# fabsig/GPBoost

Measured on AMD Instinct MI355X. Metric: neg-log-lik evals/sec, n=1000000 Vecchia(m=30) fp64, higher is better.
Workload: dtype f64

## Files before the change

### gpboost_amd/csrc/dev_common.h

```cpp
#pragma once
#include <hip/hip_runtime.h>
#include <stdint.h>
#include <type_traits>
#include <utility>

namespace gpb {

template <int B, int E, class F>
__device__ __forceinline__ void static_for(F&& f) {
  if constexpr (B < E) {
    f(std::integral_constant<int, B>{});
    static_for<B + 1, E>(f);
  }
}
template <int B, int E, class F>
__device__ __forceinline__ void static_for_down(F&& f) {
  if constexpr (B < E) {
    f(std::integral_constant<int, E - 1>{});
    static_for_down<B, E - 1>(f);
  }
}

template <int LANE>
__device__ __forceinline__ double row_bcast(double x) {
  static_assert(LANE >= 0 && LANE < 16, "row_newbcast lane");
  double r;
  asm volatile("s_nop 1\n\tv_mov_b64_dpp %0, %1 row_newbcast:%2 row_mask:0xf bank_mask:0xf"
               : "=v"(r)
               : "v"(x), "n"(LANE));
  return r;
}
template <int LANE>
__device__ __forceinline__ void row_fnma(double& acc, double b, double own) {
  static_assert(LANE >= 0 && LANE < 16, "row_newbcast lane");
#ifdef GPB_DPP_PAD_EVERY_FMAC
  asm volatile("s_nop 1\n\tv_fmac_f64_dpp %0, -%1, %2 row_newbcast:%3 row_mask:0xf bank_mask:0xf"
               : "+v"(acc)
               : "v"(b), "v"(own), "n"(LANE));
#else
  asm volatile("v_fmac_f64_dpp %0, -%1, %2 row_newbcast:%3 row_mask:0xf bank_mask:0xf"
               : "+v"(acc)
               : "v"(b), "v"(own), "n"(LANE));
#endif
}
__device__ __forceinline__ void dpp_fence(double& a) { asm volatile("s_nop 1" : "+v"(a)); }
__device__ __forceinline__ void dpp_fence(double& a, double& b) { asm volatile("s_nop 1" : "+v"(a), "+v"(b)); }
__device__ __forceinline__ void dpp_fence(double& a, double& b, double& c) { asm volatile("s_nop 1" : "+v"(a), "+v"(b), "+v"(c)); }
__device__ __forceinline__ void dpp_fence(double& a, double& b, double& c, double& d) { asm volatile("s_nop 1" : "+v"(a), "+v"(b), "+v"(c), "+v"(d)); }
template <int CTRL>
__device__ __forceinline__ double dpp_move_f64(double v) {
  const long long b = __builtin_bit_cast(long long, v);
  int lo = (int)(b & 0xffffffffll), hi = (int)(b >> 32);
  lo = __builtin_amdgcn_update_dpp(0, lo, CTRL, 0xF, 0xF, true);
  hi = __builtin_amdgcn_update_dpp(0, hi, CTRL, 0xF, 0xF, true);
  return __builtin_bit_cast(double, ((long long)hi << 32) | (long long)(unsigned int)lo);
}
__device__ __forceinline__ double row_sum16(double v) {
  v += dpp_move_f64<0xB1>(v);
  v += dpp_move_f64<0x4E>(v);
  v += dpp_move_f64<0x141>(v);
  v += dpp_move_f64<0x140>(v);
  return v;
}
__host__ __device__ constexpr unsigned long long row_lanes_le(int j) {
  return j < 0 ? 0ull : (j >= 15 ? ~0ull : ((1ull << (j + 1)) - 1ull) * 0x0001000100010001ull);
}
__host__ __device__ constexpr unsigned long long row_lane_eq(int j) { return (1ull << j) * 0x0001000100010001ull; }
template <unsigned long long MASK>
__device__ __forceinline__ int sel_lanes(int a, int b, int tok) {
  int r;
  asm("s_mov_b32 vcc_lo, %3\n\ts_mov_b32 vcc_hi, %4\n\tv_cndmask_b32_e32 %0, %1, %2, vcc ; %5"
      : "=v"(r) : "v"(b), "v"(a), "n"((int)(unsigned)(MASK & 0xffffffffull)), "n"((int)(unsigned)(MASK >> 32)), "s"(tok) : "vcc");
  return r;
}
template <unsigned long long MASK, int A, int B>
__device__ __forceinline__ int sel_lanes_const(int tok) {
  static_assert(A >= 0 && A <= 64 && B >= 0 && B <= 64, "inline constants only");
  int r;
  asm("s_mov_b32 vcc_lo, %3\n\ts_mov_b32 vcc_hi, %4\n\tv_cndmask_b32_e64 %0, %1, %2, vcc ; %5"
      : "=v"(r) : "n"(B), "n"(A), "n"((int)(unsigned)(MASK & 0xffffffffull)), "n"((int)(unsigned)(MASK >> 32)), "s"(tok) : "vcc");
  return r;
}
template <unsigned long long MASK>
__device__ __forceinline__ void set_lanes(double& dst, double v) {
  asm volatile("s_mov_b32 exec_lo, %2\n\ts_mov_b32 exec_hi, %3\n\tv_mov_b64 %0, %1\n\ts_mov_b64 exec, -1"
               : "+v"(dst) : "v"(v), "n"((int)(unsigned)(MASK & 0xffffffffull)), "n"((int)(unsigned)(MASK >> 32)));
}
template <int LANE>
__device__ __forceinline__ double row_bcast_builtin(double x) {
  const long long v = __builtin_bit_cast(long long, x);
  int lo = (int)(v & 0xffffffffll), hi = (int)(v >> 32);
  lo = __builtin_amdgcn_update_dpp(0, lo, 0x150 + LANE, 0xf, 0xf, false);
  hi = __builtin_amdgcn_update_dpp(0, hi, 0x150 + LANE, 0xf, 0xf, false);
  const long long r = ((long long)hi << 32) | (unsigned long long)(unsigned int)lo;
  return __builtin_bit_cast(double, r);
}
#ifdef GPB_DPP_VIA_BUILTIN
#define GPB_ROW_BCAST(L, x) ::gpb::row_bcast_builtin<L>(x)
#define GPB_ROW_FNMA(L, acc, b, own) (acc) = __builtin_fma(-::gpb::row_bcast_builtin<L>(b), (own), (acc))
#else
#define GPB_ROW_BCAST(L, x) ::gpb::row_bcast<L>(x)
#define GPB_ROW_FNMA(L, acc, b, own) ::gpb::row_fnma<L>((acc), (b), (own))
#endif


__device__ __forceinline__ double fast_rcp(double x) {
  const double y0 = __builtin_amdgcn_rcp(x);
  const double e = __builtin_fma(-x, y0, 1.0);
  return __builtin_fma(y0, e, y0);
}

#ifndef GPB_EXP_TAB_SIZE
#define GPB_EXP_TAB_SIZE 256
#endif
static_assert(GPB_EXP_TAB_SIZE == 256, "exp_of_scaled is written for a 256-entry table");

enum CovType : int { kMatern05 = 0, kMatern15 = 1, kMatern25 = 2 };

constexpr double kLn2OverT = 0.0027076061740622863;
constexpr double kCoordScale = 184.6649652337873;

struct KernEval { double ev, rp; };
__device__ __forceinline__ KernEval exp_of_scaled(double d2q, const double* __restrict__ tabv) {
  const double h = __builtin_amdgcn_rsq(d2q);
  const double g = d2q * h;
  const double e = __builtin_fma(-h, g, 3.0);
  const double rp = g * e;
  const double kf = __builtin_rint(-rp);
  const double rr = -rp - kf;
  const int k = (int)kf;
  double p = __builtin_fma(rr, 2.239395190875157e-12, 3.3083026805413713e-09);
  p = __builtin_fma(p, rr, 3.6655655969101062e-06);
  p = __builtin_fma(p, rr, kLn2OverT);
  p = __builtin_fma(p, rr, 1.0);
  KernEval o;
  o.ev = __builtin_ldexp(tabv[k & (GPB_EXP_TAB_SIZE - 1)] * p, k >> 8);
  o.rp = rp;
  return o;
}
template <int COV>
__device__ __forceinline__ double matern_cov_s(double d2s, const double* __restrict__ tabv) {
  const KernEval k = exp_of_scaled(d2s, tabv);
  if constexpr (COV == kMatern05) return k.ev;
  else if constexpr (COV == kMatern15) return k.ev * __builtin_fma(k.rp, kLn2OverT, 1.0);
  else { const double r = k.rp * kLn2OverT; return k.ev * __builtin_fma(r, __builtin_fma(r, 1.0 / 3.0, 1.0), 1.0); }
}
template <int COV>
__device__ __forceinline__ double matern_cov_dlog_s(double d2s, const double* __restrict__ tabv, double& dk) {
  const KernEval k = exp_of_scaled(d2s, tabv);
  const double r = k.rp * kLn2OverT;
  if constexpr (COV == kMatern05) { dk = -r * k.ev; return k.ev; }
  else if constexpr (COV == kMatern15) { dk = -(r * r) * k.ev; return k.ev * (1.0 + r); }
  else { dk = -(1.0 / 3.0) * (r * r) * (1.0 + r) * k.ev; return k.ev * __builtin_fma(r, __builtin_fma(r, 1.0 / 3.0, 1.0), 1.0); }
}
template <int COV>
__device__ __forceinline__ double matern_dlog_range_s(double d2s, const double* __restrict__ tabv) {
  const KernEval k = exp_of_scaled(d2s, tabv);
  const double r = k.rp * kLn2OverT;
  if constexpr (COV == kMatern05) return -r * k.ev;
  else if constexpr (COV == kMatern15) return -(r * r) * k.ev;
  else return -(1.0 / 3.0) * (r * r) * __builtin_fma(1.0, r, 1.0) * k.ev;
}

}
```

### gpboost_amd/csrc/vecchia_kernels.hip

```cpp
#include <algorithm>
#include "dev_common.h"
#include "vecchia_kernels.h"

namespace gpb {

namespace {

constexpr double kDummyCoord = 1e30;

__host__ __device__ constexpr int lane_of_row(int r) { return ((r / 16) & 1) ? 15 - (r % 16) : (r % 16); }

template <int MT>
struct Layout {
  static_assert(MT >= 1 && MT <= 62, "1 <= MT <= 62");
  static_assert(MT % 16 != 15, "row MT and row MT+1 must share a register slot");
  static constexpr int R = MT + 2;
  static constexpr int NS = (R + 15) / 16;
  static constexpr int PS = MT / 16, PL = lane_of_row(MT);
  static constexpr int YS = (MT + 1) / 16, YL = lane_of_row(MT + 1);
  static constexpr int NCOL = MT + 1;
  static constexpr int PTS_BYTES32 = (NS * 16) * 32 + 16;
  static constexpr int PTS_STRIDE24 = NS * 16 + 2;
  __host__ __device__ static constexpr int cmax(int s) { return (16 * s + 15 < MT) ? 16 * s + 15 : MT; }
};

template <bool D3> struct RecT;
template <> struct RecT<true> { double x, y, z, w; __device__ __forceinline__ double zz() const { return z; } };
template <> struct RecT<false> { double x, y, w; __device__ __forceinline__ double zz() const { return 0.0; } };

template <bool D3>
__device__ __forceinline__ double sq_dist_s(double px, double py, double pz, double qx, double qy, double qz) {
  const double dx = px - qx, dy = py - qy;
  double d2 = __builtin_fma(dx, dx, 1e-300);
  d2 = __builtin_fma(dy, dy, d2);
  if constexpr (D3) {
    const double dz = pz - qz;
    d2 = __builtin_fma(dz, dz, d2);
  }
  return d2;
}

template <int MT>
__host__ __device__ constexpr int num_lower_steps() {
  using L = Layout<MT>;
  int n = 8 * L::NS * (L::NS - 1) + 15 * (L::NS / 2);
  if (L::NS & 1) { const int s = L::NS - 1; const int chi = (16 * s + 14 < MT - 1) ? 16 * s + 14 : MT - 1; n += chi - 16 * s + 1; }
  return n;
}
template <int MT, class FR, class FP, class FS>
__device__ __forceinline__ void for_each_lower_step(FR&& rect, FP&& pair, FS&& solo) {
  using L = Layout<MT>;
  constexpr int RECT_TOTAL = 8 * L::NS * (L::NS - 1);
  static_for<1, L::NS>([&](auto s_) {
    constexpr int s = decltype(s_)::value;
    static_for<0, 16 * s>([&](auto c_) { rect(s_, c_, std::integral_constant<int, 8 * s * (s - 1) + decltype(c_)::value>{}); });
  });
  static_for<0, L::NS>([&](auto s_) {
    constexpr int s = decltype(s_)::value;
    if constexpr ((s & 1) == 1) {
      static_for<0, 15>([&](auto j_) {
        constexpr int j = decltype(j_)::value;
        constexpr int cA = 16 * s + j, cB = 16 * (s - 1) + 14 - j;
        using E = std::integral_constant<int, RECT_TOTAL + 15 * (s / 2) + j>;
        if constexpr (cA <= MT - 1) pair(s_, std::integral_constant<int, cA>{}, std::integral_constant<int, s - 1>{},
                                         std::integral_constant<int, cB>{}, std::integral_constant<int, 14 - j>{}, E{});
        else solo(std::integral_constant<int, s - 1>{}, std::integral_constant<int, cB>{}, E{});
      });
    } else if constexpr (s == L::NS - 1) {
      constexpr int chi = (16 * s + 14 < MT - 1) ? 16 * s + 14 : MT - 1;
      static_for<16 * s, chi + 1>([&](auto c_) { solo(s_, c_, std::integral_constant<int, RECT_TOTAL + 15 * (L::NS / 2) + decltype(c_)::value - 16 * s>{}); });
    }
  });
}

}

constexpr unsigned long long kGranuleEmpty = ~0ull;
template <int NP>
__device__ __forceinline__ void vecchia_finish(const VecchiaKernelArgs& args, int G, double (*s_fin)[4]);

template <int MT, int MODE>
constexpr bool kRuntimeWeightedInstance() { return MODE == MODE_GRAD && MT > 30 && MT <= 40; }

template <int MT, int COV, bool D3, int MODE, bool WT>
__global__ __launch_bounds__(256, (MT > 30 && MT <= 40 && MODE != MODE_NLL) ? 2 : 1) void vecchia_point_kernel(VecchiaKernelArgs args) {
  using L = Layout<MT>;
  constexpr int NS = L::NS;
  constexpr bool kNeedSolve = (MODE != MODE_NLL);
#ifdef GPB_NLL_RIGHT_LOOKING
  constexpr bool kLeftLooking = false;
#else
  constexpr bool kLeftLooking = MT > 30 && (!kNeedSolve || NS == 3);
#endif
  constexpr bool kLeftSolve = kLeftLooking && kNeedSolve;
  constexpr int NP = (MODE == MODE_GRAD) ? GPB_NUM_PARTIALS : 3;

  using Rec = RecT<D3>;
  constexpr bool kStoreDK = (MODE == MODE_GRAD) && (MT <= 30);
  constexpr int NSTEP = num_lower_steps<MT>();
  constexpr bool kLastDkInReg = kStoreDK && D3;
  constexpr int NSTORE = kStoreDK ? (kLastDkInReg ? NSTEP - 1 : NSTEP) : 1;
  constexpr int PBYTES = D3 ? L::PTS_BYTES32 : L::PTS_STRIDE24 * (int)sizeof(Rec);
  __shared__ double s_tab[GPB_EXP_TAB_SIZE];
  __shared__ __attribute__((aligned(16))) char s_pts_raw[16 * PBYTES];
  __shared__ double s_red[GPB_NUM_PARTIALS][16];
  __shared__ double s_f0[kLeftSolve ? 16 : 1][kLeftSolve ? 256 : 1];
  constexpr bool kDgInLds = WT && (MODE == MODE_NLL) && kLeftLooking;
  __shared__ double s_dg[kDgInLds ? 16 : 1][kDgInLds ? NS * 16 : 1];
  __shared__ double s_dk[NSTORE][kStoreDK ? 256 : 1];
  static_assert(PBYTES % 16 == 0 && PBYTES >= 16 * (NS * 16), "record block: 16-byte aligned, room for the (A, b) pairs");
  __shared__ double2 s_ab[(MODE == MODE_GRAD && !kStoreDK) ? 16 : 1][(MODE == MODE_GRAD && !kStoreDK) ? NS * 16 : 1];
  double dk_last = 0.0;

  __shared__ double s_tot[GPB_NUM_PARTIALS];
  __shared__ double s_fin[GPB_NUM_PARTIALS][4];

  const int G = (int)gridDim.x - 1;
  if ((int)blockIdx.x == G) { vecchia_finish<NP>(args, G, s_fin); return; }
  const int tid0 = threadIdx.x;
  static_assert(GPB_EXP_TAB_SIZE == 256, "one table entry per thread");
  s_tab[tid0] = args.exp_tab[tid0] * args.var;
  if (tid0 < NP) s_tot[tid0] = 0.0;
  __shared__ double s_pm[16];
  __shared__ int s_pe[16];
  if (tid0 < 16) { s_pm[tid0] = 0.5; s_pe[tid0] = 1; }

  const int m = args.m;
  auto fetch_idx = [&](int grp_, int tid_, int (&out)[NS]) {
    const int g_ = tid_ >> 4, l_ = tid_ & 15;
    const long long ir = (long long)args.i_begin + (long long)grp_ * 16 + g_;
    const int ii = ir < (long long)args.i_end ? (int)ir : args.i_end - 1;
#pragma unroll
    for (int s = 0; s < NS; ++s) {
      const int r = 16 * s + ((s & 1) ? 15 - l_ : l_);
      int idx = -1;
      if (r < m) idx = args.nn[(size_t)ii * m + r];
      else if (r == MT) idx = ii;
      out[s] = idx;
    }
  };
  int nidx[NS];
  fetch_idx(blockIdx.x, tid0, nidx);
  for (int grp = blockIdx.x; grp < args.ngroups; grp += G) {
  int tid = tid0;
  asm volatile("; per-trip thread index" : "+v"(tid));
  const int g = tid >> 4;
  const int l = tid & 15;
  const long long i_raw = (long long)args.i_begin + (long long)grp * 16 + g;
  const bool active = i_raw < (long long)args.i_end;
  const int i = active ? (int)i_raw : args.i_end - 1;
  int cidx[NS];
#pragma unroll
  for (int s = 0; s < NS; ++s) cidx[s] = nidx[s];
  if (grp + G < args.ngroups) fetch_idx(grp + G, tid, nidx);
  const double sc = args.a * kCoordScale;

  const double4 ctr = args.pts[i];
  Rec own[NS];
  constexpr bool kRuntimeW = WT && kRuntimeWeightedInstance<MT, MODE>();
  const bool weighted = kRuntimeW ? (args.nug != nullptr) : WT;
  constexpr int kOwnDg = (kDgInLds || !WT) ? 1 : NS;
  double own_dg[kOwnDg];
#pragma unroll
  for (int s = 0; s < kOwnDg; ++s) own_dg[s] = 0.0;
  auto own_dg_of = [&](int s) -> double { if constexpr (kOwnDg == NS) return own_dg[s]; else { (void)s; return own_dg[0]; } };
#pragma unroll
  for (int s = 0; s < NS; ++s) {
    const int r = 16 * s + ((s & 1) ? 15 - l : l);
    const int idx = cidx[s];
    if (WT && weighted) {
      const double dgv = args.var + (idx >= 0 ? args.nug[idx] : 1.0);
      if constexpr (kDgInLds) s_dg[g][r] = dgv; else own_dg[s] = dgv;
    }
    Rec p;
    if (idx >= 0) {
      const double4 q = args.pts[idx];
      p.x = (q.x - ctr.x) * sc; p.y = (q.y - ctr.y) * sc; p.w = q.w;
      if constexpr (D3) p.z = (q.z - ctr.z) * sc;
    } else {
      p.x = kDummyCoord * (double)(r + 1); p.y = 0.0; p.w = 0.0;
      if constexpr (D3) p.z = 0.0;
    }
    own[s] = p;
    reinterpret_cast<Rec*>(s_pts_raw + g * PBYTES)[r] = p;
  }
  __syncthreads();
  const double* tabv = s_tab;
  const Rec* gp = reinterpret_cast<const Rec*>(s_pts_raw + g * PBYTES);
  int row_off[NS];
#pragma unroll
  for (int s = 0; s < NS; ++s) row_off[s] = (16 * s + ((s & 1) ? 15 - l : l)) * (int)sizeof(Rec);

  double M[NS][L::NCOL];
  auto eval_entry = [&](const Rec& o, const Rec& q, auto e_) -> double {
    const double d2 = sq_dist_s<D3>(o.x, o.y, o.zz(), q.x, q.y, q.zz());
    if constexpr (kStoreDK) {
      double dk;
      const double v = matern_cov_dlog_s<COV>(d2, tabv, dk);
      if constexpr (kLastDkInReg && decltype(e_)::value == NSTEP - 1) dk_last = dk;
      else s_dk[decltype(e_)::value][tid] = dk;
      return v;
    } else {
      return matern_cov_s<COV>(d2, tabv);
    }
  };
  if constexpr (kLeftLooking) {
    auto eval_plain = [&](const Rec& o, const Rec& q) -> double {
      return matern_cov_s<COV>(sq_dist_s<D3>(o.x, o.y, o.zz(), q.x, q.y, q.zz()), tabv);
    };
    static_for<0, MT + 1>([&](auto c_) {
      constexpr int c = decltype(c_)::value;
      constexpr int sc_ = c / 16, lc = lane_of_row(c);
      if constexpr (c < MT) {
        static_for<sc_ + 1, NS>([&](auto s_) { constexpr int s = decltype(s_)::value; M[s][c] = eval_plain(own[s], gp[c]); });
        if constexpr ((c % 16) != 15 && (sc_ & 1) == 0) {
          constexpr int j = 14 - (c - 16 * sc_);
          constexpr int sA = sc_ + 1, cA = 16 * sA + j;
          if constexpr (sA < NS && cA <= MT - 1) {
            constexpr unsigned long long MA = row_lanes_le(14 - j);
            const int ro = sel_lanes<MA>(row_off[sA], row_off[sc_], grp);
            const int co = sel_lanes_const<MA, cA, c>(grp) * (int)sizeof(Rec);
            const double v = eval_plain(*reinterpret_cast<const Rec*>(reinterpret_cast<const char*>(gp) + ro),
                                        *reinterpret_cast<const Rec*>(reinterpret_cast<const char*>(gp) + co));
            M[sA][cA] = v;
            M[sc_][c] = v;
          } else {
            M[sc_][c] = eval_plain(own[sc_], gp[c]);
          }
        }
      }
      {
        double dg;
        if constexpr (kDgInLds) dg = weighted ? s_dg[g][c] : ((c == MT) ? args.diag_i : args.diag_nn);
        else dg = weighted ? own_dg_of(sc_) : ((c == MT) ? args.diag_i : args.diag_nn);
        if constexpr (c == 16 * sc_ + 15 || c == MT) M[sc_][c] = dg;
        else set_lanes<row_lane_eq(lc)>(M[sc_][c], dg);
        set_lanes<row_lane_eq(L::YL)>(M[L::YS][c], gp[c].w);
      }
      static_for<0, c>([&](auto k_) {
        constexpr int k = decltype(k_)::value;
        static_for<sc_, NS>([&](auto s_) {
          constexpr int s = decltype(s_)::value;
          GPB_ROW_FNMA(lc, M[s][c], M[sc_][k], M[s][k]);
        });
      });
      if constexpr (c < MT) {
        const double piv = GPB_ROW_BCAST(lc, M[sc_][c]);
        const double y0 = __builtin_amdgcn_rsq(piv);
        const double e = __builtin_fma(-0.5 * piv * y0, y0, 0.5);
        const double rs = __builtin_fma(y0, e, y0);
        static_for<sc_, NS>([&](auto s_) { constexpr int s = decltype(s_)::value; M[s][c] *= rs; });
        if constexpr (kLeftSolve) set_lanes<row_lane_eq(lc)>(M[sc_][c], rs);
        static_assert(NS <= 4, "dpp_fence overloads cover four slots");
        if constexpr (NS - sc_ == 1) dpp_fence(M[sc_][c]);
        else if constexpr (NS - sc_ == 2) dpp_fence(M[sc_][c], M[sc_ + 1][c]);
        else if constexpr (NS - sc_ == 3) dpp_fence(M[sc_][c], M[sc_ + 1][c], M[sc_ + 2][c]);
        else dpp_fence(M[sc_][c], M[sc_ + 1][c], M[sc_ + 2][c], M[sc_ + 3][c]);
        if constexpr (kLeftSolve && c == 15) static_for<0, 16>([&](auto q_) { s_f0[decltype(q_)::value][tid] = M[0][decltype(q_)::value]; });
      }
    });
  } else {
  for_each_lower_step<MT>(
      [&](auto s_, auto c_, auto e_) {
        constexpr int s = decltype(s_)::value, c = decltype(c_)::value;
        M[s][c] = eval_entry(own[s], gp[c], e_);
      },
      [&](auto sA_, auto cA_, auto sB_, auto cB_, auto J_, auto e_) {
        constexpr int sA = decltype(sA_)::value, cA = decltype(cA_)::value, sB = decltype(sB_)::value,
                      cB = decltype(cB_)::value, J = decltype(J_)::value;
        constexpr unsigned long long MA = row_lanes_le(J);
        const int ro = sel_lanes<MA>(row_off[sA], row_off[sB], grp);
        const int co = sel_lanes_const<MA, cA, cB>(grp) * (int)sizeof(Rec);
        const Rec o = *reinterpret_cast<const Rec*>(reinterpret_cast<const char*>(gp) + ro);
        const Rec q = *reinterpret_cast<const Rec*>(reinterpret_cast<const char*>(gp) + co);
        const double v = eval_entry(o, q, e_);
        M[sA][cA] = v;
        M[sB][cB] = v;
      },
      [&](auto s_, auto c_, auto e_) {
        constexpr int s = decltype(s_)::value, c = decltype(c_)::value;
        M[s][c] = eval_entry(own[s], gp[c], e_);
      });
  static_for<0, NS>([&](auto s_) {
    constexpr int s = decltype(s_)::value;
    static_for<16 * s, L::cmax(s) + 1>([&](auto c_) {
      constexpr int c = decltype(c_)::value;
      double dg;
      if constexpr (kDgInLds) dg = weighted ? s_dg[g][c] : ((c == MT) ? args.diag_i : args.diag_nn);
      else dg = weighted ? own_dg_of(s) : ((c == MT) ? args.diag_i : args.diag_nn);
      if constexpr (c == 16 * s + 15 || c == MT) M[s][c] = dg;
      else set_lanes<row_lane_eq(lane_of_row(c))>(M[s][c], dg);
    });
  });
  if (l == L::YL) {
    static_for<0, MT + 1>([&](auto c_) { M[L::YS][decltype(c_)::value] = gp[decltype(c_)::value].w; });
  }

  static_for<0, MT>([&](auto k_) {
    constexpr int k = decltype(k_)::value;
    constexpr int sk = k / 16, lk = lane_of_row(k);
    if constexpr (k == 0) static_for<0, NS>([&](auto s_) { dpp_fence(M[decltype(s_)::value][0]); });
    const double piv = GPB_ROW_BCAST(lk, M[sk][k]);
    const double inv = fast_rcp(piv);
    double T[NS];
    static_for<sk, NS>([&](auto s_) { T[decltype(s_)::value] = M[decltype(s_)::value][k] * inv; });
    static_for<k + 1, MT + 1>([&](auto c_) {
      constexpr int c = decltype(c_)::value;
      constexpr int sc_ = c / 16, lc = lane_of_row(c);
      static_for<sc_, NS>([&](auto s_) {
        constexpr int s = decltype(s_)::value;
        GPB_ROW_FNMA(lc, M[s][c], M[sc_][k], T[s]);
      });
    });
    if constexpr (kNeedSolve) static_for<sk, NS>([&](auto s_) { M[decltype(s_)::value][k] = T[decltype(s_)::value]; });
  });
  }

  const double Dv = GPB_ROW_BCAST(L::PL, M[L::PS][MT]);
  const double uv = GPB_ROW_BCAST(L::YL, M[L::YS][MT]);
  const double Dinv = 1.0 / Dv;

  double red[GPB_NUM_PARTIALS];
#pragma unroll
  for (int t = 0; t < GPB_NUM_PARTIALS; ++t) red[t] = 0.0;
  red[GPB_P_LOGDET] = Dv;
  red[GPB_P_QUAD] = uv * uv * Dinv;
  red[GPB_P_BAD] = (Dv > 0.0) ? 0.0 : 1.0;

  if constexpr (kNeedSolve) {
    constexpr bool kLaneX = MT > 30;
    double X[kLaneX ? 1 : MT];
    double xa[NS], xb[NS];
    if constexpr (kLeftSolve) {
      static_assert(NS == 3 && L::PS == 2 && L::YS == 2, "kLeftSolve: three slots, the point's and the response row in the last one");
#pragma unroll
      for (int s = 0; s < NS; ++s) { xa[s] = 0.0; xb[s] = 0.0; }
      static_for_down<0, MT>([&](auto k_) {
        constexpr int k = decltype(k_)::value;
        constexpr int sk = k / 16, lk = lane_of_row(k);
        constexpr unsigned long long kKeep = (sk & 1) ? row_lanes_le(14 - (k % 16)) : ~row_lanes_le(k % 16);
        double own_col;
        if constexpr (sk == 0) own_col = s_f0[k][tid]; else own_col = M[sk][k];
        double ta = own_col * xa[sk], tb = own_col * xb[sk];
        set_lanes<~kKeep>(ta, 0.0);
        set_lanes<~kKeep>(tb, 0.0);
        static_for<sk + 1, NS>([&](auto s_) {
          constexpr int s = decltype(s_)::value;
          ta = __builtin_fma(M[s][k], xa[s], ta);
          tb = __builtin_fma(M[s][k], xb[s], tb);
        });
        ta = row_sum16(ta); tb = row_sum16(tb);
        const double rk = GPB_ROW_BCAST(lk, own_col);
        const double la = GPB_ROW_BCAST(L::PL, M[L::PS][k]);
        const double lb = GPB_ROW_BCAST(L::YL, M[L::YS][k]);
        set_lanes<row_lane_eq(lk)>(xa[sk], (la - ta) * rk);
        set_lanes<row_lane_eq(lk)>(xb[sk], (lb - tb) * rk);
      });
    } else if constexpr (kLaneX) {
#pragma unroll
      for (int s = 0; s < NS; ++s) { xa[s] = 0.0; xb[s] = 0.0; }
      static_for_down<0, MT>([&](auto k_) {
        constexpr int k = decltype(k_)::value;
        constexpr int sk = k / 16, lk = lane_of_row(k);
        constexpr unsigned long long kKeep = (sk & 1) ? row_lanes_le(14 - (k % 16)) : ~row_lanes_le(k % 16);
        double ta = M[sk][k] * xa[sk], tb = M[sk][k] * xb[sk];
        set_lanes<~kKeep>(ta, 0.0);
        set_lanes<~kKeep>(tb, 0.0);
        static_for<sk + 1, NS>([&](auto s_) {
          constexpr int s = decltype(s_)::value;
          ta = __builtin_fma(M[s][k], xa[s], ta);
          tb = __builtin_fma(M[s][k], xb[s], tb);
        });
        ta = row_sum16(ta); tb = row_sum16(tb);
        const double la = GPB_ROW_BCAST(L::PL, M[L::PS][k]);
        const double lb = GPB_ROW_BCAST(L::YL, M[L::YS][k]);
        set_lanes<row_lane_eq(lk)>(xa[sk], la - ta);
        set_lanes<row_lane_eq(lk)>(xb[sk], lb - tb);
      });
    } else {
    static_for<0, MT>([&](auto k_) { X[decltype(k_)::value] = M[L::PS][decltype(k_)::value]; });
    static_for<0, MT>([&](auto k_) { static_for<0, NS>([&](auto s_) { if constexpr (decltype(k_)::value <= L::cmax(decltype(s_)::value)) dpp_fence(M[decltype(s_)::value][decltype(k_)::value]); }); });
    static_for_down<0, MT>([&](auto j_) {
      constexpr int j = decltype(j_)::value;
      constexpr int sj = j / 16, lj = lane_of_row(j);
      static_for_down<0, j>([&](auto k_) {
        constexpr int k = decltype(k_)::value;
        GPB_ROW_FNMA(lj, X[k], M[sj][k], X[j]);
      });
    });
    }
    if constexpr (MODE == MODE_FACTOR) {
      if constexpr (kLaneX) {
        if (active) {
          double* Arow = args.A + (size_t)i * m;
#pragma unroll
          for (int s = 0; s < NS; ++s) { const int r = 16 * s + ((s & 1) ? 15 - l : l); if (r < m) Arow[r] = xa[s]; }
        }
      } else {
      if (active && l == L::PL) {
        double* Arow = args.A + (size_t)i * m;
        static_for<0, MT>([&](auto k_) {
          constexpr int k = decltype(k_)::value;
          if (k < m) Arow[k] = X[k];
        });
      }
      }
      if (active && l == 0) { args.D[i] = Dv; args.u[i] = uv; }
    }
    if constexpr (MODE == MODE_GRAD) {
      asm volatile("" ::: "memory");
      double2* gab = kStoreDK ? reinterpret_cast<double2*>(s_pts_raw + g * PBYTES) : &s_ab[g][0];
      if constexpr (kLaneX) {
#pragma unroll
        for (int s = 0; s < NS; ++s) {
          const int r = 16 * s + ((s & 1) ? 15 - l : l);
          gab[r] = r < MT ? make_double2(xa[s], xb[s]) : (r == MT ? make_double2(-1.0, 0.0) : make_double2(0.0, 0.0));
        }
      } else {
      if (l == L::PL) { static_for<0, MT>([&](auto k_) { gab[decltype(k_)::value].x = X[decltype(k_)::value]; }); gab[MT].x = -1.0; gab[MT + 1].x = 0.0; }
      if (l == L::YL) { static_for<0, MT>([&](auto k_) { gab[decltype(k_)::value].y = X[decltype(k_)::value]; }); gab[MT].y = 0.0; gab[MT + 1].y = 0.0; }
      if (l == 0) { for (int r = MT + 2; r < NS * 16; ++r) gab[r] = make_double2(0.0, 0.0); }
      }
      __syncthreads();
      double2 abr[NS];
      int ab_off[NS];
      double sAA = 0.0, sbA = 0.0;
      static_for<0, NS>([&](auto s_) {
        constexpr int s = decltype(s_)::value;
        const int r = 16 * s + ((s & 1) ? 15 - l : l);
        abr[s] = gab[r]; ab_off[s] = r * (int)sizeof(double2);
        const double nr = weighted ? own_dg_of(s) - args.var : 1.0;
        if (r < MT) { sAA = __builtin_fma(nr * abr[s].x, abr[s].x, sAA); sbA = __builtin_fma(nr * abr[s].y, abr[s].x, sbA); }
      });
      double accD = 0.0, accU = 0.0;
      auto accumulate = [&](double dk, const double2& r_, const double2& c_) {
        accD = __builtin_fma(dk * r_.x, c_.x, accD);
        accU = __builtin_fma(dk, __builtin_fma(r_.y, c_.x, c_.y * r_.x), accU);
      };
      auto dk_of = [&](auto e_, const Rec& o, const Rec& q) -> double {
        if constexpr (kStoreDK) {
          if constexpr (kLastDkInReg && decltype(e_)::value == NSTEP - 1) return dk_last;
          else return s_dk[decltype(e_)::value][tid];
        } else {
          return matern_dlog_range_s<COV>(sq_dist_s<D3>(o.x, o.y, o.zz(), q.x, q.y, q.zz()), tabv);
        }
      };
      for_each_lower_step<MT>(
          [&](auto s_, auto c_, auto e_) {
            constexpr int s = decltype(s_)::value, c = decltype(c_)::value;
            if constexpr (kStoreDK) accumulate(dk_of(e_, own[s], gp[c]), abr[s], gab[c]);
            else accumulate(dk_of(e_, *reinterpret_cast<const Rec*>(reinterpret_cast<const char*>(gp) + row_off[s]), gp[c]), abr[s], gab[c]);
          },
          [&](auto sA_, auto cA_, auto sB_, auto cB_, auto J_, auto e_) {
            constexpr int sA = decltype(sA_)::value, cA = decltype(cA_)::value, sB = decltype(sB_)::value,
                          cB = decltype(cB_)::value, J = decltype(J_)::value;
            constexpr unsigned long long MA = row_lanes_le(J);
            const int ci = sel_lanes_const<MA, cA, cB>(grp);
            double dk;
            if constexpr (kStoreDK) dk = dk_of(e_, own[0], own[0]);
            else {
              const int ro = sel_lanes<MA>(row_off[sA], row_off[sB], grp);
              dk = dk_of(e_, *reinterpret_cast<const Rec*>(reinterpret_cast<const char*>(gp) + ro),
                         *reinterpret_cast<const Rec*>(reinterpret_cast<const char*>(gp) + ci * (int)sizeof(Rec)));
            }
            const int ao = sel_lanes<MA>(ab_off[sA], ab_off[sB], grp);
            accumulate(dk, *reinterpret_cast<const double2*>(reinterpret_cast<const char*>(gab) + ao), gab[ci]);
          },
          [&](auto s_, auto c_, auto e_) {
            constexpr int s = decltype(s_)::value, c = decltype(c_)::value;
            static_assert((s & 1) == 0, "solo steps only occur in even slots");
            double dk;
            if constexpr (kStoreDK) dk = dk_of(e_, own[s], gp[c]);
            else dk = dk_of(e_, *reinterpret_cast<const Rec*>(reinterpret_cast<const char*>(gp) + row_off[s]), gp[c]);
            set_lanes<row_lanes_le(c - 16 * s)>(dk, 0.0);
            accumulate(dk, abr[s], gab[c]);
          });
#pragma unroll
      for (int off = 8; off >= 1; off >>= 1) {
        accD += __shfl_xor(accD, off, 16);
        accU += __shfl_xor(accU, off, 16);
        sAA += __shfl_xor(sAA, off, 16);
        sbA += __shfl_xor(sbA, off, 16);
      }
      const double up = uv * Dinv;
      double nug_i = args.nugget;
      if (WT && weighted) nug_i = args.nug[i];
      const double dD_var = Dv - nug_i - sAA;
      const double uk_var = -sbA;
      const double dD_rng = 2.0 * accD;
      const double uk_rng = accU;
      red[GPB_P_G1_VAR] = uk_var * up - 0.5 * up * up * dD_var;
      red[GPB_P_G2_VAR] = 0.5 * Dinv * dD_var;
      red[GPB_P_G1_RNG] = uk_rng * up - 0.5 * up * up * dD_rng;
      red[GPB_P_G2_RNG] = 0.5 * Dinv * dD_rng;
    }
  }

  if (l == 0) {
#pragma unroll
    for (int t = 0; t < NP; ++t) s_red[t][g] = active ? red[t] : (t == GPB_P_LOGDET ? 1.0 : 0.0);
  }
  __syncthreads();
  if (tid < 16) {
    const double dv = s_red[GPB_P_LOGDET][tid];
    const double p = s_pm[tid] * __builtin_amdgcn_frexp_mant(dv);
    s_pm[tid] = (dv > 0.0) ? __builtin_amdgcn_frexp_mant(p) : __builtin_nan("");
    s_pe[tid] += __builtin_amdgcn_frexp_exp(dv) + __builtin_amdgcn_frexp_exp(p);
  } else if (tid >= 64 && tid < 64 + NP && tid - 64 != GPB_P_LOGDET) {
    const int t = tid - 64;
    double acc = 0.0;
#pragma unroll
    for (int q = 0; q < 16; ++q) acc += s_red[t][q];
    s_tot[t] += acc;
  }
  }
  const int tid = tid0;
  __syncthreads();
  if (tid < 16) s_red[GPB_P_LOGDET][tid] = log(s_pm[tid]) + (double)s_pe[tid] * 0.693147180559945309417232121458;
  __syncthreads();
  if (tid == 0) {
    double acc = 0.0;
#pragma unroll
    for (int q = 0; q < 16; ++q) acc += s_red[GPB_P_LOGDET][q];
    s_tot[GPB_P_LOGDET] = acc;
  }
  __syncthreads();

  if (tid < NP)
    __hip_atomic_store(reinterpret_cast<unsigned long long*>(args.partials + (size_t)tid * G + blockIdx.x),
                       (unsigned long long)__double_as_longlong(s_tot[tid]), __ATOMIC_RELAXED, __HIP_MEMORY_SCOPE_AGENT);
}

template <int NP>
__device__ __forceinline__ void vecchia_finish(const VecchiaKernelArgs& args, int G, double (*s_fin)[4]) {
  const int tid = threadIdx.x;
#pragma unroll
  for (int t = 0; t < NP; ++t) {
    double acc = 0.0, comp = 0.0;
    unsigned long long* base = reinterpret_cast<unsigned long long*>(args.partials + (size_t)t * G);
    constexpr int kBatch = 8;
    for (int b0 = tid; b0 < G; b0 += 256 * kBatch) {
      unsigned long long raw[kBatch];
#pragma unroll
      for (int q = 0; q < kBatch; ++q) {
        const int b = b0 + 256 * q;
        raw[q] = b < G ? __hip_atomic_load(base + b, __ATOMIC_RELAXED, __HIP_MEMORY_SCOPE_AGENT) : 0ull;
      }
#pragma unroll
      for (int q = 0; q < kBatch; ++q) {
        const int b = b0 + 256 * q;
        if (b >= G) break;
        while (raw[q] == kGranuleEmpty) {
          __builtin_amdgcn_s_sleep(8);
          raw[q] = __hip_atomic_load(base + b, __ATOMIC_RELAXED, __HIP_MEMORY_SCOPE_AGENT);
        }
        __hip_atomic_store(base + b, kGranuleEmpty, __ATOMIC_RELAXED, __HIP_MEMORY_SCOPE_AGENT);
        const double v = __longlong_as_double((long long)raw[q]) - comp;
        const double tmp = acc + v;
        comp = (tmp - acc) - v;
        acc = tmp;
      }
    }
#pragma unroll
    for (int off = 32; off >= 1; off >>= 1) acc += __shfl_xor(acc, off, 64);
    if ((tid & 63) == 0) s_fin[t][tid >> 6] = acc;
  }
  __syncthreads();
  if (tid < NP) {
    const double v = (s_fin[tid][0] + s_fin[tid][1]) + (s_fin[tid][2] + s_fin[tid][3]);
    args.out[tid] = v;
    if (args.out_user) args.out_user[tid == GPB_P_LOGDET ? 1 : (tid == GPB_P_QUAD ? 0 : tid)] = v;
    if (args.out_host) __hip_atomic_store(reinterpret_cast<unsigned long long*>(args.out_host + tid), (unsigned long long)__double_as_longlong(v),
                                          __ATOMIC_RELAXED, __HIP_MEMORY_SCOPE_SYSTEM);
  }
}


#ifdef GPB_INSTANTIATE_MT
#ifndef GPB_INSTANTIATE_MODE
#error "define GPB_INSTANTIATE_MODE (0 nll, 1 factor, 2 grad) together with GPB_INSTANTIATE_MT"
#endif
template <int MT, int COV, bool D3, bool WT>
static int persistent_grid_uncapped(const VecchiaKernelArgs& args) {
  auto kern = vecchia_point_kernel<MT, COV, D3, GPB_INSTANTIATE_MODE, WT>;
  static int cached_dev = -1, per_dev = 0;
  int dev = 0;
  if (hipGetDevice(&dev) != hipSuccess) return args.ngroups;
  if (dev != cached_dev) {
    int occ = 0, cus = 0;
    if (hipOccupancyMaxActiveBlocksPerMultiprocessor(&occ, kern, 256, 0) != hipSuccess || occ < 1) occ = 1;
    if (hipDeviceGetAttribute(&cus, hipDeviceAttributeMultiprocessorCount, dev) != hipSuccess || cus < 1) cus = 256;
    per_dev = occ * cus; cached_dev = dev;
    (void)hipGetLastError();
  }
  const int auto_rounds = (int)std::max(1LL, std::min(8LL, ((long long)args.ngroups + 2LL * per_dev) / (4LL * per_dev)));
  const long long slots = (long long)per_dev * auto_rounds;
  if (args.ngroups <= slots) return args.ngroups;
  const int trips = (int)((args.ngroups + slots - 1) / slots);
  return (args.ngroups + trips - 1) / trips;
}
template <int MT, int COV, bool D3, bool WT>
static int persistent_grid(const VecchiaKernelArgs& args) {
  const int workers = persistent_grid_uncapped<MT, COV, D3, WT>(args);
  return args.max_workers > 0 ? std::min(workers, args.max_workers) : workers;
}
template <int MT, bool D3>
static hipError_t launch_cov(int cov, const VecchiaKernelArgs& args, int nblocks, hipStream_t st) {
  (void)nblocks;
  switch (cov) {
#define GPB_LAUNCH_COV(C) \
  if (args.nug || kRuntimeWeightedInstance<MT, GPB_INSTANTIATE_MODE>()) hipLaunchKernelGGL((vecchia_point_kernel<MT, C, D3, GPB_INSTANTIATE_MODE, true>), dim3(persistent_grid<MT, C, D3, true>(args) + 1), dim3(256), 0, st, args); \
  else hipLaunchKernelGGL((vecchia_point_kernel<MT, C, D3, GPB_INSTANTIATE_MODE, false>), dim3(persistent_grid<MT, C, D3, false>(args) + 1), dim3(256), 0, st, args); \
  break
    case kMatern05: GPB_LAUNCH_COV(kMatern05);
    case kMatern15: GPB_LAUNCH_COV(kMatern15);
    case kMatern25: GPB_LAUNCH_COV(kMatern25);
#undef GPB_LAUNCH_COV
    default: return hipErrorInvalidValue;
  }
  return hipGetLastError();
}
#define GPB_CAT4_(a, b, c, d) a##b##c##d
#define GPB_CAT4(a, b, c, d) GPB_CAT4_(a, b, c, d)
hipError_t GPB_CAT4(launch_vecchia_mt, GPB_INSTANTIATE_MT, _mode, GPB_INSTANTIATE_MODE)(bool d3, int cov, const VecchiaKernelArgs& args,
                                                                                      int nblocks, hipStream_t st) {
  return d3 ? launch_cov<GPB_INSTANTIATE_MT, true>(cov, args, nblocks, st)
            : launch_cov<GPB_INSTANTIATE_MT, false>(cov, args, nblocks, st);
}
#else
#define GPB_CASE(MTV)                                                                                   \
  hipError_t launch_vecchia_mt##MTV##_mode0(bool, int, const VecchiaKernelArgs&, int, hipStream_t);       \
  hipError_t launch_vecchia_mt##MTV##_mode1(bool, int, const VecchiaKernelArgs&, int, hipStream_t);       \
  hipError_t launch_vecchia_mt##MTV##_mode2(bool, int, const VecchiaKernelArgs&, int, hipStream_t);
GPB_MT_CASES
#undef GPB_CASE

int vecchia_padded_m(int m) {
  const int sizes[] = {GPB_MT_LIST};
  for (int s : sizes) if (m <= s) return s;
  return -1;
}

hipError_t launch_vecchia_point_kernel(int mode, int cov, bool d3, const VecchiaKernelArgs& args, hipStream_t st) {
  const int npts = args.i_end - args.i_begin;
  if (npts <= 0) return hipErrorInvalidValue;
  const int nblocks = (npts + 15) / 16;
  if (args.ngroups != nblocks || !args.out) return hipErrorInvalidValue;
  const int mt = vecchia_padded_m(args.m);
  switch (mt) {
#define GPB_CASE(MTV)                                                                       \
  case MTV:                                                                                   \
    if (mode == MODE_NLL) return launch_vecchia_mt##MTV##_mode0(d3, cov, args, nblocks, st);  \
    if (mode == MODE_FACTOR) return launch_vecchia_mt##MTV##_mode1(d3, cov, args, nblocks, st); \
    if (mode == MODE_GRAD) return launch_vecchia_mt##MTV##_mode2(d3, cov, args, nblocks, st);  \
    return hipErrorInvalidValue;
    GPB_MT_CASES
#undef GPB_CASE
    default: return hipErrorInvalidValue;
  }
}

#endif

}
```

Baseline: 1082.

## Trim per-trip overhead in two-slot Vecchia kernel: pair LDS table, lean indexing, pivot tweaks

For the two-slot (MT<=30) right-looking path, the kernel now precomputes per-lane LDS addresses for the symmetric pair steps in a shared table, replacing the per-step lane-select address math. It also simplifies the neighbor-index and center-point fetch arithmetic using 32-bit offsets from the group start. The first pivot's reciprocal is hoisted as a uniform value when unweighted, and the DPP broadcast padding nop is dropped for middle pivots. Together these aim to cut scalar/VALU instructions in the hot factorization loop. The trade-off is extra LDS use and a dependence on the hardware DPP hazard rules, where dropping the nop could be unsafe.

Result: faster. 1123 (median of 6 runs) (+3.8%).

```diff
diff --git a/gpboost_amd/csrc/dev_common.h b/gpboost_amd/csrc/dev_common.h
--- a/gpboost_amd/csrc/dev_common.h
+++ b/gpboost_amd/csrc/dev_common.h
@@ -31,6 +31,19 @@
   return r;
 }
 template <int LANE>
+__device__ __forceinline__ double row_bcast_nopad(double x) {
+  static_assert(LANE >= 0 && LANE < 16, "row_newbcast lane");
+#ifdef GPB_DPP_PAD_EVERY_FMAC
+  return row_bcast<LANE>(x);
+#else
+  double r;
+  asm volatile("v_mov_b64_dpp %0, %1 row_newbcast:%2 row_mask:0xf bank_mask:0xf"
+               : "=v"(r)
+               : "v"(x), "n"(LANE));
+  return r;
+#endif
+}
+template <int LANE>
 __device__ __forceinline__ void row_fnma(double& acc, double b, double own) {
   static_assert(LANE >= 0 && LANE < 16, "row_newbcast lane");
 #ifdef GPB_DPP_PAD_EVERY_FMAC
@@ -61,6 +74,15 @@
   v += dpp_move_f64<0x141>(v);
   v += dpp_move_f64<0x140>(v);
   return v;
+}
+using LdsDouble = __attribute__((address_space(3))) double;
+__device__ __forceinline__ const LdsDouble* lds_doubles_at(unsigned addr) {
+#if defined(__HIP_DEVICE_COMPILE__)
+  return (const LdsDouble*)addr;
+#else
+  (void)addr;
+  return nullptr;
+#endif
 }
 __host__ __device__ constexpr unsigned long long row_lanes_le(int j) {
   return j < 0 ? 0ull : (j >= 15 ? ~0ull : ((1ull << (j + 1)) - 1ull) * 0x0001000100010001ull);
@@ -97,9 +119,11 @@
 }
 #ifdef GPB_DPP_VIA_BUILTIN
 #define GPB_ROW_BCAST(L, x) ::gpb::row_bcast_builtin<L>(x)
+#define GPB_ROW_BCAST_NOPAD(L, x) ::gpb::row_bcast_builtin<L>(x)
 #define GPB_ROW_FNMA(L, acc, b, own) (acc) = __builtin_fma(-::gpb::row_bcast_builtin<L>(b), (own), (acc))
 #else
 #define GPB_ROW_BCAST(L, x) ::gpb::row_bcast<L>(x)
+#define GPB_ROW_BCAST_NOPAD(L, x) ::gpb::row_bcast_nopad<L>(x)
 #define GPB_ROW_FNMA(L, acc, b, own) ::gpb::row_fnma<L>((acc), (b), (own))
 #endif
 
diff --git a/gpboost_amd/csrc/vecchia_kernels.hip b/gpboost_amd/csrc/vecchia_kernels.hip
--- a/gpboost_amd/csrc/vecchia_kernels.hip
+++ b/gpboost_amd/csrc/vecchia_kernels.hip
@@ -96,6 +96,8 @@
   constexpr int NP = (MODE == MODE_GRAD) ? GPB_NUM_PARTIALS : 3;
 
   using Rec = RecT<D3>;
+  constexpr bool kLeanTrip = (NS == 2);
+  static_assert(!kLeanTrip || !kLeftLooking, "two slots: MT <= 30, right-looking");
   constexpr bool kStoreDK = (MODE == MODE_GRAD) && (MT <= 30);
   constexpr int NSTEP = num_lower_steps<MT>();
   constexpr bool kLastDkInReg = kStoreDK && D3;
@@ -111,6 +113,9 @@
   static_assert(PBYTES % 16 == 0 && PBYTES >= 16 * (NS * 16), "record block: 16-byte aligned, room for the (A, b) pairs");
   __shared__ double2 s_ab[(MODE == MODE_GRAD && !kStoreDK) ? 16 : 1][(MODE == MODE_GRAD && !kStoreDK) ? NS * 16 : 1];
   double dk_last = 0.0;
+  constexpr bool kPairTab = kLeanTrip && MODE != MODE_GRAD;
+  constexpr int NPAIR = kPairTab ? ((MT - 16 < 15) ? MT - 16 : 15) : 0;
+  __shared__ unsigned short s_pair[NPAIR > 0 ? NPAIR : 1][2][NPAIR > 0 ? 256 : 1];
 
   __shared__ double s_tot[GPB_NUM_PARTIALS];
   __shared__ double s_fin[GPB_NUM_PARTIALS][4];
@@ -124,38 +129,83 @@
   __shared__ double s_pm[16];
   __shared__ int s_pe[16];
   if (tid0 < 16) { s_pm[tid0] = 0.5; s_pe[tid0] = 1; }
-
+  if constexpr (NPAIR > 0) {
+    const int g0 = tid0 >> 4, l0 = tid0 & 15;
+    static_for<0, NPAIR>([&](auto j_) {
+      constexpr int j = decltype(j_)::value;
+      const bool upper = l0 <= 14 - j;
+      const int row = upper ? 31 - l0 : l0, col = upper ? 16 + j : 14 - j;
+      s_pair[j][0][tid0] = (unsigned short)(size_t)(s_pts_raw + g0 * PBYTES + row * (int)sizeof(Rec));
+      s_pair[j][1][tid0] = (unsigned short)(size_t)(s_pts_raw + g0 * PBYTES + col * (int)sizeof(Rec));
+    });
+  }
+
+  constexpr bool kFirstInv = !WT && kLeanTrip;
+  double inv_first = 0.0;
+  if constexpr (kFirstInv) {
+    const long long b = __builtin_bit_cast(long long, fast_rcp(args.diag_nn));
+    const int lo = __builtin_amdgcn_readfirstlane((int)(b & 0xffffffffll)), hi = __builtin_amdgcn_readfirstlane((int)(b >> 32));
+    inv_first = __builtin_bit_cast(double, ((long long)hi << 32) | (long long)(unsigned int)lo);
+  }
   const int m = args.m;
+  auto group_first = [&](int grp_) -> long long { return (long long)args.i_begin + (long long)grp_ * 16; };
+  auto group_last = [&](int grp_) -> int { const long long rem = (long long)args.i_end - group_first(grp_) - 1; return rem < 15 ? (int)rem : 15; };
   auto fetch_idx = [&](int grp_, int tid_, int (&out)[NS]) {
     const int g_ = tid_ >> 4, l_ = tid_ & 15;
-    const long long ir = (long long)args.i_begin + (long long)grp_ * 16 + g_;
-    const int ii = ir < (long long)args.i_end ? (int)ir : args.i_end - 1;
-#pragma unroll
-    for (int s = 0; s < NS; ++s) {
-      const int r = 16 * s + ((s & 1) ? 15 - l_ : l_);
-      int idx = -1;
-      if (r < m) idx = args.nn[(size_t)ii * m + r];
-      else if (r == MT) idx = ii;
-      out[s] = idx;
+    if constexpr (kLeanTrip) {
+      const long long first = group_first(grp_);
+      const int last = group_last(grp_);
+      const int gc = g_ < last ? g_ : last;
+      const char* rows = reinterpret_cast<const char*>(args.nn + (size_t)first * (size_t)m);
+#pragma unroll
+      for (int s = 0; s < NS; ++s) {
+        const int r = 16 * s + ((s & 1) ? 15 - l_ : l_);
+        int idx = -1;
+        if (r < m) idx = *reinterpret_cast<const int*>(rows + ((unsigned)gc * (unsigned)m + (unsigned)r) * 4u);
+        else if (r == MT) idx = (int)first + gc;
+        out[s] = idx;
+      }
+    } else {
+      const long long ir = (long long)args.i_begin + (long long)grp_ * 16 + g_;
+      const int ii = ir < (long long)args.i_end ? (int)ir : args.i_end - 1;
+#pragma unroll
+      for (int s = 0; s < NS; ++s) {
+        const int r = 16 * s + ((s & 1) ? 15 - l_ : l_);
+        int idx = -1;
+        if (r < m) idx = args.nn[(size_t)ii * m + r];
+        else if (r == MT) idx = ii;
+        out[s] = idx;
+      }
     }
   };
   int nidx[NS];
-  fetch_idx(blockIdx.x, tid0, nidx);
+  if (!kLeanTrip || (int)blockIdx.x < args.ngroups) fetch_idx(blockIdx.x, tid0, nidx);
   for (int grp = blockIdx.x; grp < args.ngroups; grp += G) {
   int tid = tid0;
   asm volatile("; per-trip thread index" : "+v"(tid));
   const int g = tid >> 4;
   const int l = tid & 15;
-  const long long i_raw = (long long)args.i_begin + (long long)grp * 16 + g;
-  const bool active = i_raw < (long long)args.i_end;
-  const int i = active ? (int)i_raw : args.i_end - 1;
+  bool active;
+  int i, g_in = 0;
+  if constexpr (kLeanTrip) {
+    const int g_last = group_last(grp);
+    active = g <= g_last;
+    g_in = active ? g : g_last;
+    i = (int)group_first(grp) + g_in;
+  } else {
+    const long long i_raw = (long long)args.i_begin + (long long)grp * 16 + g;
+    active = i_raw < (long long)args.i_end;
+    i = active ? (int)i_raw : args.i_end - 1;
+  }
   int cidx[NS];
 #pragma unroll
   for (int s = 0; s < NS; ++s) cidx[s] = nidx[s];
   if (grp + G < args.ngroups) fetch_idx(grp + G, tid, nidx);
   const double sc = args.a * kCoordScale;
 
-  const double4 ctr = args.pts[i];
+  double4 ctr;
+  if constexpr (kLeanTrip) ctr = *reinterpret_cast<const double4*>(reinterpret_cast<const char*>(args.pts + group_first(grp)) + (unsigned)g_in * 32u);
+  else ctr = args.pts[i];
   Rec own[NS];
   constexpr bool kRuntimeW = WT && kRuntimeWeightedInstance<MT, MODE>();
   const bool weighted = kRuntimeW ? (args.nug != nullptr) : WT;
@@ -178,6 +228,7 @@
       p.x = (q.x - ctr.x) * sc; p.y = (q.y - ctr.y) * sc; p.w = q.w;
       if constexpr (D3) p.z = (q.z - ctr.z) * sc;
     } else {
+      if constexpr (kLeanTrip) asm volatile("; dummy rows");
       p.x = kDummyCoord * (double)(r + 1); p.y = 0.0; p.w = 0.0;
       if constexpr (D3) p.z = 0.0;
     }
@@ -269,10 +320,20 @@
         constexpr int sA = decltype(sA_)::value, cA = decltype(cA_)::value, sB = decltype(sB_)::value,
                       cB = decltype(cB_)::value, J = decltype(J_)::value;
         constexpr unsigned long long MA = row_lanes_le(J);
-        const int ro = sel_lanes<MA>(row_off[sA], row_off[sB], grp);
-        const int co = sel_lanes_const<MA, cA, cB>(grp) * (int)sizeof(Rec);
-        const Rec o = *reinterpret_cast<const Rec*>(reinterpret_cast<const char*>(gp) + ro);
-        const Rec q = *reinterpret_cast<const Rec*>(reinterpret_cast<const char*>(gp) + co);
+        Rec o, q;
+        if constexpr (kPairTab) {
+          static_assert(sA == 1 && sB == 0 && J == 14 - (cA - 16) && cB == J, "s_pair is filled for this enumeration of the pair steps");
+          const LdsDouble* po = lds_doubles_at(s_pair[cA - 16][0][tid]);
+          const LdsDouble* pq = lds_doubles_at(s_pair[cA - 16][1][tid]);
+          o.x = po[0]; o.y = po[1]; q.x = pq[0]; q.y = pq[1];
+          if constexpr (D3) { o.z = po[2]; q.z = pq[2]; }
+          o.w = 0.0; q.w = 0.0;
+        } else {
+          const int ro = sel_lanes<MA>(row_off[sA], row_off[sB], grp);
+          const int co = sel_lanes_const<MA, cA, cB>(grp) * (int)sizeof(Rec);
+          o = *reinterpret_cast<const Rec*>(reinterpret_cast<const char*>(gp) + ro);
+          q = *reinterpret_cast<const Rec*>(reinterpret_cast<const char*>(gp) + co);
+        }
         const double v = eval_entry(o, q, e_);
         M[sA][cA] = v;
         M[sB][cB] = v;
@@ -300,8 +361,10 @@
     constexpr int k = decltype(k_)::value;
     constexpr int sk = k / 16, lk = lane_of_row(k);
     if constexpr (k == 0) static_for<0, NS>([&](auto s_) { dpp_fence(M[decltype(s_)::value][0]); });
-    const double piv = GPB_ROW_BCAST(lk, M[sk][k]);
-    const double inv = fast_rcp(piv);
+    double inv;
+    if constexpr (kFirstInv && k == 0) inv = inv_first;
+    else if constexpr (kLeanTrip && k >= 1 && k <= MT - 3) inv = fast_rcp(GPB_ROW_BCAST_NOPAD(lk, M[sk][k]));
+    else inv = fast_rcp(GPB_ROW_BCAST(lk, M[sk][k]));
     double T[NS];
     static_for<sk, NS>([&](auto s_) { T[decltype(s_)::value] = M[decltype(s_)::value][k] * inv; });
     static_for<k + 1, MT + 1>([&](auto c_) {
```
